# oppo-us-research/PoP-Net

Measured on AMD Instinct MI355X. Metric: depth-frames/sec end-to-end (480x640), higher is better.
Workload: dtype bf16

## Files before the change

popnet_amd/csrc/api.hip:

```cpp
#pragma clang fp contract(off)
#include <cmath>
#include <cstdio>
#include <cstdlib>
#include <cstring>
#include "pn_internal.h"
#include "preproc_pixel.h"

template <typename TIN>
__global__ void preprocess_kernel(const TIN *__restrict__ depth, float *__restrict__ out, int B, int H, int W, int S,
                                  double scale_x, double scale_y, float dmax, float mean, float stdv) {
    const unsigned pix = blockIdx.x * blockDim.x + threadIdx.x;
    if (pix >= (unsigned)(S * S)) return;
    const int b = blockIdx.y;
    const int dy = (int)(pix / (unsigned)S);
    const int dx = (int)(pix - (unsigned)dy * (unsigned)S);
    const size_t gid = (size_t)b * S * S + pix;

    out[gid] = pn_preproc_pixel(depth + (size_t)b * H * W, H, W, dy, dx, scale_x, scale_y, dmax, mean, stdv);
}

PnSwitches pn_read_switches() {
    auto set = [](const char *name) { return getenv(name) != nullptr; };
    auto num = [](const char *name, int unset) { const char *e = getenv(name); return e ? atoi(e) : unset; };
    auto is = [](const char *name, const char *value) { const char *e = getenv(name); return e && !strcmp(e, value); };
    PnSwitches s;
    s.no_conv3 = set("POPNET_NO_CONV3");
    s.conv3_rpg8 = set("POPNET_CONV3_RPG8");
    s.conv3_pt14 = num("POPNET_CONV3_PT14", 0);
    s.conv3_nbuf2 = set("POPNET_CONV3_NBUF2");
    s.generic_c64_off = num("POPNET_GENERIC_C64", 1) == 0;
    if (set("POPNET_CONV4")) s.conv4 = num("POPNET_CONV4", 0) == 0 ? 0 : 1;
    s.no_mix = set("POPNET_NO_MIX");
    s.no_bblock = set("POPNET_NO_BBLOCK");
    s.bblock_x3 = num("POPNET_BBLOCK_X3", 0) != 0;
    s.bb64_static = set("POPNET_BB64_STATIC");
    s.bb64_halves = num("POPNET_BB64_HALVES", 1) == 2 ? 2 : 1;
    s.no_tailfuse = set("POPNET_NO_TAILFUSE");
    s.no_poolfuse = set("POPNET_NO_POOLFUSE");
    s.no_stempool = set("POPNET_NO_STEMPOOL");
    s.no_embed3 = set("POPNET_NO_EMBED3");
    s.train_x3_wide = set("POPNET_TRAIN_X3_WIDE");
    s.train_wgrad_novec = set("POPNET_TRAIN_WGRAD_NOVEC");
    s.trainx_one_stream = num("POPNET_TRAINX_STREAMS", 0) == 1;
    s.trainx_stem_handover = set("POPNET_TRAINX_STEM_HANDOVER");
    s.trainx_stem_gather = is("POPNET_TRAINX_STEM_FWD", "gather");
    s.trainx_stem_bn_separate = is("POPNET_TRAINX_STEM_BN", "separate");
    s.trainx_stem_depth = num("POPNET_TRAINX_STEM_DEPTH", 2);
    s.trainx_pack_gather = is("POPNET_TRAINX_PACK", "gather");
    s.trainx_legacy_wgrad = is("POPNET_TRAINX_WGRAD", "legacy");
    return s;
}

extern "C" {

int pn_abi_version(void) { return PN_ABI_VERSION; }
int pn_build_experiments(void) { return 0; }

pn_ctx *pn_create(int device_id) {
    pn_ctx *ctx = new pn_ctx();
    ctx->device = device_id;
    int ndev = 0;
    hipError_t e = hipGetDeviceCount(&ndev);
    if (e != hipSuccess || device_id < 0 || device_id >= ndev) {
        char buf[256];
        snprintf(buf, sizeof buf, "pn_create: device %d not available (%d devices, %s)", device_id, ndev,
                 hipGetErrorString(e));
        ctx->err = buf;
        ctx->device = -1;
        return ctx;
    }
    hipDeviceProp_t prop;
    if (hipGetDeviceProperties(&prop, device_id) == hipSuccess) ctx->num_cus = prop.multiProcessorCount;
    return ctx;
}

void pn_destroy(pn_ctx *ctx) {
    if (!ctx) return;
    if (ctx->parse_ws) (void)hipFree(ctx->parse_ws);
    pn_parse_big_free(ctx);
    if (ctx->train_ws) (void)hipFree(ctx->train_ws);
    for (void *p : ctx->train_ws_retired) (void)hipFree(p);
    for (auto &e : ctx->train_packs) (void)hipFree(e.buf);
    if (ctx->train_pack_table) (void)hipFree(ctx->train_pack_table);
    delete ctx;
}

int pn_last_error(pn_ctx *ctx, char *buf, size_t buf_len) {
    if (!ctx) return 0;
    if (buf && buf_len) {
        size_t n = ctx->err.size() < buf_len - 1 ? ctx->err.size() : buf_len - 1;
        memcpy(buf, ctx->err.data(), n);
        buf[n] = 0;
    }
    return (int)ctx->err.size();
}

int pn_preprocess(pn_ctx *ctx, const void *depth_dev, int depth_dtype, int B, int H, int W, float *out_dev, int S,
                  float depth_max, float depth_mean, float depth_std, void *hip_stream) {
    if (!ctx) return PN_ERR_INVALID;
    if (ctx->device < 0) return pn_set_error(ctx, PN_ERR_STATE, "context has no device");
    if (!depth_dev || !out_dev || B < 1 || H < 2 || W < 2 || S < 1)
        return pn_set_error(ctx, PN_ERR_INVALID, "pn_preprocess: bad arguments");
    if (W == 2 * S && H == 2 * S)
        return pn_set_error(ctx, PN_ERR_UNSUPPORTED, "pn_preprocess: %dx%d -> %d is an exact 2x decimation, where cv2.resize(INTER_LINEAR) runs INTER_AREA instead: not built", W, H, S);
    const double inv_x = (double)S / (double)W, inv_y = (double)S / (double)H;
    const double scale_x = 1.0 / inv_x, scale_y = 1.0 / inv_y;
    if (B > 65535 || (size_t)S * S > 0x7fffffffu) return pn_set_error(ctx, PN_ERR_INVALID, "pn_preprocess: batch or output size out of range");
    dim3 grid((unsigned)(((size_t)S * S + 255) / 256), (unsigned)B), block(256);
    hipStream_t s = (hipStream_t)hip_stream;
// ... 31 lines not shown
```

popnet_amd/csrc/conv_mfma.hip:

```cpp
#include "pn_internal.h"

int pn_cfg_couts(int cfg) {
    switch (cfg) {
        case PN_CFG_C128: return 128;
        case PN_CFG_C64: return 64;
        case PN_CFG_C64W: return 64;
        case PN_CFG_C32: return 32;
        default: return 16;
    }
}


int pn_cfg_pixels(int cfg) { return cfg == PN_CFG_C128 ? 112 : (cfg == PN_CFG_C64W ? 224 : 128); }

size_t pn_conv_lds_bytes(int prec, int ks, int stride, int pitch, int R) {
    size_t pixb = prec == PN_PREC_BF16 ? 128 : 256;
    size_t rows = (size_t)(R - 1) * stride + ks;
    return rows * pitch * pixb;
}

int pn_launch_conv_part0(pn_ctx *ctx, const ConvLaunch &L, hipStream_t stream);
int pn_launch_conv_part1(pn_ctx *ctx, const ConvLaunch &L, hipStream_t stream);
int pn_launch_conv_part2(pn_ctx *ctx, const ConvLaunch &L, hipStream_t stream);
int pn_launch_conv_part3(pn_ctx *ctx, const ConvLaunch &L, hipStream_t stream);

int pn_launch_conv(pn_ctx *ctx, const ConvLaunch &L, hipStream_t stream) {
    int rc;
    if (L.kern == 4) return pn_launch_conv4(ctx, L, stream);
    if (L.kern == 3) return pn_launch_conv3(ctx, L, stream);
    if ((rc = pn_launch_conv_part0(ctx, L, stream)) != 1) return rc;
    if ((rc = pn_launch_conv_part1(ctx, L, stream)) != 1) return rc;
    if ((rc = pn_launch_conv_part2(ctx, L, stream)) != 1) return rc;
    if ((rc = pn_launch_conv_part3(ctx, L, stream)) != 1) return rc;
    return pn_set_error(ctx, PN_ERR_UNSUPPORTED, "no conv kernel for prec=%d ks=%d stride=%d pitch=%d cfg=%d", L.prec, L.ks,
                        L.stride, L.pitch, L.cfg);
}

int pn_conv_stage_maxpx(int prec, int ks, int stride, int pitch, int cfg) {
    if (cfg == PN_CFG_C64W) return 0;
    const int maxpx = stride != 1 ? 0 : (ks == 1 ? 128 : (pitch <= 32 ? 192 : (pitch <= 64 ? 288 : 360)));
    const int nch = prec == PN_PREC_BF16 ? 8 : 16;
    const int raw = (maxpx * nch + 255) / 256;
    return raw <= 12 ? maxpx : 0;
}
```

popnet_amd/csrc/conv_plan.h:

```cpp
#pragma once
#include <algorithm>
#include "pn_internal.h"

struct ConvGeom {
    int kern = 0, cfg = 0, pitch = 0, R = 0, Wt = 0;
    int wc = 0, wp = 0, nbuf = 0, pt = 7, rpg = 4;
};

inline int pn_pick_pitch(int cols) {
    const int classes[4] = {16, 32, 64, 120};
    for (int c : classes)
        if (cols <= c) return c;
    return -1;
}

inline int pn_pick_cfg(int cout) {
    if (cout % 128 == 0) return PN_CFG_C128;
    if (cout >= 64) return PN_CFG_C64;
    if (cout <= 16) return PN_CFG_C16;
    return PN_CFG_C32;
}

inline void pn_plan_conv_kernel(int prec, int max_batch, int num_cus, int H, int W, int cout, int ks, int stride, int cin_chunks, int wc_min, int nbuf_min,
                                int k4_level, const PnSwitches &sw, ConvGeom &g) {
    g.cfg = pn_pick_cfg(cout);
    {
        int segs = 0, wt = 0, rows = 0, rpg = 4;
        double best = 0;
        for (int sg = (W + 29) / 30; sg <= (W + 15) / 16; ++sg) {
            const int w = (W + sg - 1) / sg;
            for (int gg : {4, 8}) {
                if (gg == 8 && !(w <= 14 && ks == 3 && cout > 64 && sw.conv3_rpg8)) continue;
                const int r = std::min(std::min(H, gg), 112 / w);
                const double util = r * ((double)W / sg) / 112.0;
                if (util > best + 1e-9) { best = util; segs = sg; wt = w; rows = r; rpg = gg; }
            }
        }
        if (prec == PN_PREC_BF16 && stride == 1 && (ks == 3 || ks == 1) && best >= 0.75 && cout > 32 && !sw.no_conv3) {
            g.kern = 3;
            g.wc = std::max(cout > 64 ? 4 : (cout > 32 ? 2 : 1), wc_min);
            const long tiles112 = (long)max_batch * ((H + rows - 1) / rows) * segs;
            g.wp = (g.wc == 2 && rows == 4 && rpg == 4 && tiles112 * ((cout + 63) / 64) >= 1536) ? 2 : 1;
            g.rpg = rpg;
            if (g.wp == 2 && ks == 3 && cin_chunks == 1 && sw.conv3_pt14 == 1) { g.wp = 1; g.pt = 14; g.rpg = 8; }
            if (sw.conv3_pt14 == 2 && ks == 3 && g.wc == 4 && g.wp == 1 && rpg == 4 && rows == 4 && H >= 8) { g.pt = 14; g.rpg = 8; }
            const int hr = rpg * g.wp + ks - 1, ngw = (8 * (hr / 2) + g.wc * g.wp - 1) / (g.wc * g.wp);
            g.nbuf = ((cin_chunks > 1 || nbuf_min == 2) && ks == 3 && ngw <= 18 && sw.conv3_nbuf2) ? 2 : 1;
            g.Wt = wt;
            g.R = std::min(H, rows * g.wp * (g.pt / 7));
            if (ks == 3 && g.wp == 1 && g.pt == 7 && g.rpg == 4 && cout >= 64 && k4_level)
                g.kern = 4;
        }
    }
    if (g.kern == 0 && prec == PN_PREC_BF16 && g.cfg == PN_CFG_C128 && stride == 1) {
        const long blocks128 = (long)max_batch * ((H * W + 111) / 112) * (cout / 128);
        if (blocks128 < num_cus && !sw.generic_c64_off) g.cfg = PN_CFG_C64;
    }
}

inline int pn_plan_conv_tiles(int prec, int H, int W, int ks, int stride, ConvGeom &g, const char **why) {
    const int Ho = (H + 2 * (ks / 2) - ks) / stride + 1, Wo = (W + 2 * (ks / 2) - ks) / stride + 1;
    if (g.kern == 3 || g.kern == 4) { g.pitch = 32; return PN_OK; }
    if (g.cfg == PN_CFG_C64 && ks == 3 && stride == 1 && Wo >= 48 && (long)Ho * Wo >= 2048) g.cfg = PN_CFG_C64W;
    const int BP = pn_cfg_pixels(g.cfg);
    const int wt_cap = std::min(BP, (120 - ks) / stride + 1);
    const int segs = (Wo + wt_cap - 1) / wt_cap;
    g.Wt = (Wo + segs - 1) / segs;
    g.R = std::max(1, std::min(Ho, BP / g.Wt));
    {
        const int maxpx = pn_conv_stage_maxpx(prec, ks, stride, pn_pick_pitch((g.Wt - 1) * stride + ks), g.cfg);
        while (maxpx > 0 && g.R > 1 && ((g.R - 1) * stride + ks) * ((g.Wt - 1) * stride + ks) > maxpx) --g.R;
        if (maxpx > 0 && ((g.R - 1) * stride + ks) * ((g.Wt - 1) * stride + ks) > maxpx) { *why = "halo tile exceeds the staging capacity"; return PN_ERR_UNSUPPORTED; }
    }
    g.pitch = pn_pick_pitch((g.Wt - 1) * stride + ks);
    if (g.pitch < 0) { *why = "halo width has no pitch class"; return PN_ERR_UNSUPPORTED; }
    return PN_OK;
}
```

popnet_amd/csrc/net.hip:

```cpp
#include <cmath>
#include <cstdarg>
#include <cstdio>
#include <algorithm>
#include <cstdlib>
#include <cstring>
#include <map>
#include <memory>
#include <vector>
#include "pn_internal.h"
#include "conv_plan.h"
#include "preproc_pixel.h"

namespace {

struct HostTensor {
    std::vector<int64_t> shape;
    std::vector<float> data;
    size_t numel() const { return data.size(); }
};

struct Buf {
    void *p = nullptr;
    int H = 0, W = 0, C = 0;
    int plane = 0;
// ... 109 lines not shown
int dev_alloc(pn_net *n, void **p, size_t bytes, bool zero) {
    PN_HIP_CHECK(n->ctx, hipMalloc(p, bytes));
    n->dev_allocs.push_back(*p);
    if (zero) PN_HIP_CHECK(n->ctx, hipMemset(*p, 0, bytes));
    return PN_OK;
}

int new_buf(pn_net *n, int H, int W, int C) {
    Buf b;
    b.H = H; b.W = W; b.plane = C; b.C = n->x3 ? 2 * C : C;
    n->bufs.push_back(b);
    return (int)n->bufs.size() - 1;
}

int prepare_conv(pn_net *n, ConvSpec &cs) {
    pn_ctx *ctx = n->ctx;
    const HostTensor *w = find_t(n, cs.w + ".weight");
    if (!w || w->shape.size() != 4)
        return pn_set_error(ctx, PN_ERR_INVALID, "missing conv weight %s.weight", cs.w.c_str());
    const int cout = (int)w->shape[0], cin_ref = (int)w->shape[1], wks = (int)w->shape[2];
    const int ks = cs.embed3 ? 3 : wks;
    if ((cs.embed3 ? wks != 1 : wks != cs.ks) || (int)w->shape[3] != wks || ks != cs.ks)
        return pn_set_error(ctx, PN_ERR_INVALID, "%s.weight: kernel %dx%d, expected %d", cs.w.c_str(), wks, (int)w->shape[3], cs.embed3 ? 1 : cs.ks);
    cs.cout = cout;
    std::vector<int> map = cs.cin_map;
    if (map.empty()) {
        map.resize(cin_ref);
        for (int i = 0; i < cin_ref; ++i) map[i] = i;
    }
    for (int m : map)
        if (m >= cin_ref)
            return pn_set_error(ctx, PN_ERR_INVALID, "%s: input-channel map exceeds Cin=%d", cs.w.c_str(), cin_ref);
    std::vector<int> wsel;
    if (n->x3) {
        const int pc = n->bufs[cs.in_buf].plane;
        if (cs.in_coff != 0 || (int)map.size() > pc)
            return pn_set_error(ctx, PN_ERR_UNSUPPORTED, "%s: bf16x3 convolutions read whole buffers", cs.w.c_str());
        map.resize(pc, -1);
        std::vector<int> m3;
        for (int pl = 0; pl < 3; ++pl)
            for (int i = 0; i < pc; ++i) { m3.push_back(map[i]); wsel.push_back(pl == 2 ? 1 : 0); }
        map.swap(m3);
    }
    const int cin_pad = ((int)map.size() + 63) / 64 * 64;
    map.resize(cin_pad, -1);
    wsel.resize(cin_pad, 0);
    cs.cin_chunks = cin_pad / 64;
    cs.cin = cin_ref;

    std::vector<double> scale(cout, 1.0), shift(cout, 0.0);
    const HostTensor *bias = find_t(n, cs.w + ".bias");
    if (bias && (int)bias->numel() != cout) return pn_set_error(ctx, PN_ERR_INVALID, "%s.bias: bad size", cs.w.c_str());
    for (int o = 0; o < cout; ++o) shift[o] = bias ? bias->data[o] : 0.0;
    if (!cs.bn.empty()) {
        const HostTensor *g = find_t(n, cs.bn + ".weight"), *be = find_t(n, cs.bn + ".bias");
        const HostTensor *mu = find_t(n, cs.bn + ".running_mean"), *var = find_t(n, cs.bn + ".running_var");
        if (!g || !be || !mu || !var || (int)g->numel() != cout || (int)be->numel() != cout ||
            (int)mu->numel() != cout || (int)var->numel() != cout)
            return pn_set_error(ctx, PN_ERR_INVALID, "missing/ill-shaped BatchNorm tensors %s.*", cs.bn.c_str());
        for (int o = 0; o < cout; ++o) {
            double s = (double)g->data[o] / std::sqrt((double)var->data[o] + 1e-5);
            scale[o] = s;
            shift[o] = (shift[o] - (double)mu->data[o]) * s + (double)be->data[o];
        }
    }

    auto wval = [&](int co, int idx, int tap) -> float {
        const int ci = map[idx];
        if (co >= cout || ci < 0) return 0.f;
        if (cs.embed3 && tap != 4) return 0.f;
        const float v = (float)((double)w->data[cs.embed3 ? (size_t)co * cin_ref + ci : ((size_t)co * cin_ref + ci) * (ks * ks) + tap] * scale[co]);
        if (!n->x3) return v;
        uint32_t hb = (uint32_t)f32_to_bf16(v) << 16;
        float hi;
        memcpy(&hi, &hb, 4);
        return wsel[idx] ? v - hi : hi;
    };

    ConvGeom geo;
    geo.pt = cs.pt; geo.rpg = cs.rpg;
    {
        const Buf &ib0 = n->bufs[cs.in_buf];
        pn_plan_conv_kernel(n->prec, n->max_batch, n->ctx->num_cus, ib0.H, ib0.W, cout, ks, cs.stride, cs.cin_chunks, cs.wc_min, cs.nbuf_min, cs.k4_level, n->sw, geo);
    }
    cs.cfg = geo.cfg; cs.kern = geo.kern; cs.wc = geo.wc; cs.wp = geo.wp; cs.nbuf = geo.nbuf; cs.pt = geo.pt; cs.rpg = geo.rpg; cs.Wt = geo.Wt; cs.R = geo.R;
    const int BC = cs.kern == 4 ? 128 : (cs.kern == 3 ? cs.wc * 32 : pn_cfg_couts(cs.cfg));
    const int cout_pad = (cout + BC - 1) / BC * BC;
    const int ctiles = cout_pad / 16;
    const int KK = ks * ks;
    const int ksteps = cs.cin_chunks * KK * 2;
    const size_t fragb = n->prec == PN_PREC_BF16 ? 1024 : 2048;
    const size_t bytes = cs.kern == 4 ? (size_t)(cout_pad / 128) * (ksteps + 3) * 8192
                                      : (size_t)ctiles * ksteps * fragb + 5 * fragb;
    std::vector<unsigned char> host(bytes, 0);
    uint16_t *h16 = reinterpret_cast<uint16_t *>(host.data());
    float *h32 = reinterpret_cast<float *>(host.data());
    if (cs.kern == 4) {
        for (int cbk = 0; cbk < cout_pad / 128; ++cbk)
            for (int hh = 0; hh < cs.cin_chunks * 2; ++hh)
                for (int tap = 0; tap < KK; ++tap)
                    for (int t = 0; t < 8; ++t)
                        for (int lane = 0; lane < 64; ++lane) {
                            const int co = cbk * 128 + pn_conv_row_channel(t, lane & 15, 4), q = lane >> 4;
                            const size_t base = ((((size_t)cbk * (ksteps + 3) + (size_t)hh * KK + tap) * 8 + t) * 64 + lane) * 8;
                            for (int j = 0; j < 8; ++j) h16[base + j] = f32_to_bf16(wval(co, hh * 32 + 8 * q + j, tap));
                        }
    } else
    for (int ct = 0; ct < ctiles; ++ct)
        for (int chunk = 0; chunk < cs.cin_chunks; ++chunk)
            for (int sub = 0; sub < 2; ++sub)
                for (int tap = 0; tap < KK; ++tap) {
                    const size_t kstep = (size_t)(chunk * 2 + sub) * KK + tap;
                    const size_t frag = (size_t)ct * ksteps + kstep;
                    for (int lane = 0; lane < 64; ++lane) {
                        const int co = pn_conv_row_channel(ct, lane & 15, cs.kern == 3 ? 2 : pn_cfg_ct(cs.cfg)), q = lane >> 4;
                        for (int j = 0; j < 8; ++j) {
                            const float v = wval(co, chunk * 64 + sub * 32 + 8 * q + j, tap);
                            if (n->prec == PN_PREC_BF16) h16[(frag * 64 + lane) * 8 + j] = f32_to_bf16(v);
                            else h32[frag * 512 + (size_t)(j >> 2) * 256 + lane * 4 + (j & 3)] = v;
                        }
                    }
                }
    if (int rc = dev_alloc(n, &cs.wpack, bytes, false)) return rc;
    PN_HIP_CHECK(ctx, hipMemcpy(cs.wpack, host.data(), bytes, hipMemcpyHostToDevice));
    std::vector<float> hb(cout_pad, 0.f);
    for (int o = 0; o < cout; ++o) hb[o] = (float)shift[o];
    if (int rc = dev_alloc(n, (void **)&cs.bias, hb.size() * 4, false)) return rc;
    PN_HIP_CHECK(ctx, hipMemcpy(cs.bias, hb.data(), hb.size() * 4, hipMemcpyHostToDevice));

    const Buf &ib = n->bufs[cs.in_buf];
    const int Ho = (ib.H + 2 * (ks / 2) - ks) / cs.stride + 1, Wo = (ib.W + 2 * (ks / 2) - ks) / cs.stride + 1;
    {
        const char *why = "";
        if (int rc = pn_plan_conv_tiles(n->prec, ib.H, ib.W, ks, cs.stride, geo, &why)) return pn_set_error(ctx, rc, "%s: %s", cs.w.c_str(), why);
        cs.cfg = geo.cfg; cs.pitch = geo.pitch; cs.Wt = geo.Wt; cs.R = geo.R;
    }
    cs.flops = 2.0 * Ho * Wo * (double)cout * cin_ref * (cs.embed3 ? 1 : KK);
    if (cs.out_buf >= 0) {
        const Buf &ob = n->bufs[cs.out_buf];
        if (ob.H != Ho || ob.W != Wo) return pn_set_error(ctx, PN_ERR_INVALID, "%s: output buffer is %dx%d, conv gives %dx%d", cs.w.c_str(), ob.H, ob.W, Ho, Wo);
    }
    return PN_OK;
}

int add_conv(pn_net *n, const std::string &w, const std::string &bn, int ks, int stride, int in_buf, int in_coff,
             int out_buf, int out_coff, int act, int res_buf = -1, int nchw_slot = -1,
             std::vector<int> cin_map = std::vector<int>()) {
    ConvSpec cs;
    cs.w = w; cs.bn = bn; cs.ks = ks; cs.stride = stride;
    cs.in_buf = in_buf; cs.in_coff = in_coff;
    cs.out_buf = out_buf; cs.out_coff = out_coff;
    cs.res_buf = res_buf; cs.act = act; cs.nchw_slot = nchw_slot;
    cs.cin_map = std::move(cin_map);
    n->convs.push_back(cs);
    return (int)n->convs.size() - 1;
}

void harmonize_level(pn_net *n, const std::vector<int> &ids) {
    {
        bool k4 = false;
        for (int id : ids) {
            const ConvSpec &c = n->convs[id];
            const HostTensor *w = find_t(n, c.w + ".weight");
            if (w && w->shape.size() == 4 && c.ks == 3 && c.stride == 1 && w->shape[0] >= 64 && (n->x3 || std::max<int64_t>(w->shape[1], (int64_t)c.cin_map.size()) > 64)) k4 = true;
        }
        long blocks = 0;
// ... 475 lines not shown
    for (auto &st : n->steps) {
        if (st.type != Step::CONV) continue;
        const ConvSpec &c0 = n->convs[st.conv_ids[0]];
        const int BC = c0.kern == 4 ? 128 : (c0.kern == 3 ? c0.wc * 32 : pn_cfg_couts(c0.cfg));
        st.host_probs.clear();
        int max_blocks = 0;
        bool two_bufs = false, has_tail = false, pool_tail = false;
        for (int id : st.conv_ids) {
            const ConvSpec &cs = n->convs[id];
            const Buf &ib = n->bufs[cs.in_buf];
            ConvProblem P;
            memset(&P, 0, sizeof P);
            const size_t es = n->esize();
            (void)es;
            P.in = ib.p;
            P.wpack = cs.wpack;
            P.bias = cs.bias;
            P.B = B; P.H = ib.H; P.W = ib.W;
            P.Ho = (ib.H + 2 * (cs.ks / 2) - cs.ks) / cs.stride + 1;
            P.Wo = (ib.W + 2 * (cs.ks / 2) - cs.ks) / cs.stride + 1;
            P.cin_chunks = cs.cin_chunks;
            P.in_cs = ib.C; P.in_coff = cs.in_coff;
            if (n->x3 && ib.plane % 64)
                return pn_set_error(n->ctx, PN_ERR_UNSUPPORTED, "bf16x3: input plane of %d channels is not a multiple of 64 (the K loop wraps to the hi plane per 64-channel chunk)", ib.plane);
            P.in_wrap = n->x3 ? 2 * (ib.plane / 64) : (1 << 20);
            P.cout = cs.cout;
            if (cs.out_buf >= 0) { P.out = n->bufs[cs.out_buf].p; P.out_cs = n->bufs[cs.out_buf].C; P.out_coff = cs.out_coff; P.split = n->x3 ? n->bufs[cs.out_buf].plane : 0; }
            if (cs.res_buf >= 0) { P.res = n->bufs[cs.res_buf].p; P.res_cs = n->bufs[cs.res_buf].C; P.res_coff = cs.res_coff; P.res_split = n->x3 ? n->bufs[cs.res_buf].plane : 0; }
            if (cs.nchw_slot >= 0) P.out_nchw = n->nchw_ptr[cs.nchw_slot];
            P.act = cs.act;
            P.yolo_naf = 5 + 3 * n->num_parts;
            P.R = cs.R;
            P.Wt = cs.Wt;
            P.tiles_x = (P.Wo + cs.Wt - 1) / cs.Wt;
            P.tiles_per_img = ((P.Ho + cs.R - 1) / cs.R) * P.tiles_x;
            P.cout_blocks = (cs.cout + BC - 1) / BC;
            P.nblocks = B * P.tiles_per_img * P.cout_blocks;
            if (cs.kern == 4) P.nblocks = ((B * P.tiles_per_img + 1) / 2) * P.cout_blocks;
            P.ksteps = cs.cin_chunks * cs.ks * cs.ks * 2;
            P.ks = cs.ks;
            P.lds_buf_bytes = (int)pn_conv_lds_bytes(n->prec, cs.ks, cs.stride, cs.pitch, cs.R);
            P.lds_two = (cs.cin_chunks > 1 && 2 * (size_t)P.lds_buf_bytes <= 160 * 1024) ? 1 : 0;
            P.in_zero_off = (unsigned)((size_t)n->max_batch * ib.H * ib.W * ib.C * es);
            if (cs.pool_tail) {
                const Buf &pb = n->bufs[cs.pool_out_buf];
                P.tiles_x = (pb.W + 6) / 7;
                P.tiles_per_img = ((pb.H + 2) / 3) * P.tiles_x;
                P.nblocks = B * P.tiles_per_img * P.cout_blocks;
                P.tail_out = pb.p; P.tail_out_cs = pb.C; P.tail_out_coff = cs.pool_out_coff;
                P.tail_split = n->x3 ? pb.plane : 0;
                P.out = nullptr;
                pool_tail = true;
            }
            if (cs.tail_conv >= 0) {
                const ConvSpec &tb = n->convs[cs.tail_conv];
                P.tail_w = cs.tail_wpack; P.tail_bias = cs.tail_bias; P.tail_cout = tb.cout; P.tail_act = tb.act;
                if (tb.out_buf >= 0) { P.tail_out = n->bufs[tb.out_buf].p; P.tail_out_cs = n->bufs[tb.out_buf].C; P.tail_out_coff = tb.out_coff; }
                if (tb.nchw_slot >= 0) P.tail_nchw = n->nchw_ptr[tb.nchw_slot];
                P.out = nullptr;
                has_tail = true;
            }
            if (P.lds_two) two_bufs = true;
            max_blocks = std::max(max_blocks, P.nblocks);
            st.host_probs.push_back(P);
        }
        st.launch.prec = n->prec;
        st.launch.ks = c0.ks; st.launch.stride = c0.stride; st.launch.pitch = c0.pitch; st.launch.cfg = c0.cfg;
        st.launch.nprob = (int)st.host_probs.size();
        st.launch.max_blocks = max_blocks;
        st.launch.lds_bytes = pn_conv_lds_bytes(n->prec, c0.ks, c0.stride, c0.pitch, c0.R) * (two_bufs ? 2 : 1);
        st.launch.kern = c0.kern; st.launch.wc = c0.wc; st.launch.wp = c0.wp; st.launch.nbuf = c0.nbuf; st.launch.pt = c0.pt; st.launch.rpg = c0.rpg;
        if (c0.kern == 3) st.launch.lds_bytes = pn_conv3_lds_bytes(c0.ks, c0.wp, c0.nbuf, c0.rpg);
        st.launch.tail = (c0.kern == 3 && has_tail) ? 1 : (c0.kern == 3 && pool_tail) ? 2 : 0;
        st.launch.mix = 0;
        if (c0.kern == 3) {
            for (int id : st.conv_ids) {
                const ConvSpec &cs = n->convs[id];
                if (cs.ks != c0.ks || (cs.tail_conv >= 0) != (c0.tail_conv >= 0)) st.launch.mix = 1;
                st.launch.lds_bytes = std::max(st.launch.lds_bytes, pn_conv3_lds_bytes(cs.ks, cs.wp, cs.nbuf, cs.rpg));
            }
            if (st.launch.tail == 1) st.launch.lds_bytes = std::max<size_t>(st.launch.lds_bytes, 4 * 7 * 1024 + 1024);
            if (st.launch.tail == 2 && n->x3) st.launch.lds_bytes = std::max<size_t>(st.launch.lds_bytes, 2 * 4 * 7 * 1024);
        }
        if (c0.kern == 4) st.launch.lds_bytes = 0;
        st.launch.probs_dev = st.dev_probs;
        PN_HIP_CHECK(n->ctx, hipMemcpyAsync(st.dev_probs, st.host_probs.data(), st.host_probs.size() * sizeof(ConvProblem),
                                            hipMemcpyHostToDevice, stream));
    }
    n->last_B = B;
    for (int i = 0; i < 4; ++i) n->last_nchw[i] = n->nchw_ptr[i];
    return PN_OK;
}

std::string step_label(const pn_net *n, const Step &st) {
    if (st.type == Step::STEM) {
        if (st.stem_pool_buf >= 0) return "stem7x7_pool_kernel";
        if (st.stem_cin > 1) return "conv2d_forward+nchw_relu_to_nhwc_kernel";
        if (n->prec == PN_PREC_F32) return "stem7x7_kernel";
        return n->x3 ? "stem7x7_mfma_kernel<x3>" : "stem7x7_mfma_kernel";
    }
    if (st.type == Step::POOL) return pn_pool_kernel_label(st.mode, n->x3);
    if (st.type == Step::BBLOCK) return n->x3 ? "bb64x3_kernel" : "bb64_kernel";
    const ConvSpec &c0 = n->convs[st.conv_ids[0]];
    bool mix = false;
    for (int id : st.conv_ids) {
        const ConvSpec &cs = n->convs[id];
        if (cs.ks != c0.ks || (cs.tail_conv >= 0) != (c0.tail_conv >= 0)) mix = true;
    }
    return pn_conv_kernel_label(n->prec, c0.kern, mix, c0.ks, c0.stride, c0.pitch, c0.cfg, c0.wc, c0.wp, c0.nbuf, c0.pt, c0.rpg);
}

int run_forward(pn_net *n, const float *x, int B, hipStream_t stream, int nsteps = -1) {
    pn_ctx *ctx = n->ctx;
    if (!n->finalized) return pn_set_error(ctx, PN_ERR_STATE, "pn_net_finalize has not been called");
    if (B < 1 || B > n->max_batch) return pn_set_error(ctx, PN_ERR_INVALID, "batch %d outside [1, %d]", B, n->max_batch);
    bool dirty = B != n->last_B;
    for (int i = 0; i < 4; ++i) dirty |= n->nchw_ptr[i] != n->last_nchw[i];
    if (dirty) {
        if (n->locked)
            return pn_set_error(ctx, PN_ERR_STATE, "net is locked at batch %d (pn_net_lock): a forward with another batch size or other output buffers would rewrite descriptors a captured graph still reads", n->last_B);
        if (int rc = refresh_problems(n, B, stream)) return rc;
    }
    if (n->tickets_suspect) {
        for (auto &st : n->steps)
            if (st.type == Step::BBLOCK && st.bb_tickets) PN_HIP_CHECK(ctx, hipMemsetAsync(st.bb_tickets, 0, 256, stream));
        n->tickets_suspect = false;
    }
    for (size_t si = 0; si < n->steps.size(); ++si) {
        if ((int)si == nsteps) break;
        Step &st = n->steps[si];
        int rc = PN_OK;
        pn_net::ProfRec *pr = nullptr;
        if (n->profiling) {
            if (n->prof_used == n->prof.size()) {
                pn_net::ProfRec r;
                PN_HIP_CHECK(ctx, hipEventCreate(&r.a));
                PN_HIP_CHECK(ctx, hipEventCreate(&r.b));
                n->prof.push_back(r);
            }
            pr = &n->prof[n->prof_used++];
            pr->kind = (int)st.type;
            pr->flops = 0;
            pr->label.clear();
            if (st.type == Step::CONV) {
                for (int id : st.conv_ids) pr->flops += n->convs[id].flops * B;
                pr->label = step_label(n, st);
            }
            if (st.type == Step::BBLOCK) {
                pr->kind = (int)Step::CONV;
                pr->flops = (n->convs[st.bb_a].flops + n->convs[st.bb_b].flops) * B;
                pr->label = step_label(n, st);
            }
            PN_HIP_CHECK(ctx, hipEventRecord(pr->a, stream));
        }
        if (st.type == Step::STEM && st.stem_pool_buf >= 0) {
            const Buf &ob = n->bufs[st.out_buf], &pb = n->bufs[st.stem_pool_buf];
            rc = pn_launch_stem_pool(ctx, x, st.stem_wfrag, st.stem_b, pb.p, B, n->in_h, n->in_w, ob.H, ob.W, pb.C, stream, n->frame_src.frames ? &n->frame_src : nullptr);
        } else if (st.type == Step::STEM && st.stem_cin > 1) {
            const Buf &ob = n->bufs[st.out_buf];
            if (n->frame_src.frames) return pn_set_error(ctx, PN_ERR_UNSUPPORTED, "the frames-in forward takes single-channel depth frames (input_dim = 1)");
            rc = pn_conv2d_forward(ctx, x, st.stem_w, st.stem_b, st.stem_scratch, B, st.stem_cin, n->in_h, n->in_w, 64, 7, 2, 3, 0, (void *)stream);
            if (!rc) rc = pn_launch_nchw_relu_to_nhwc(ctx, n->prec, st.stem_scratch, ob.p, B, ob.H, ob.W, 64, ob.C, n->x3 ? ob.plane : 0, stream);
        } else if (st.type == Step::STEM) {
            const Buf &ob = n->bufs[st.out_buf];
            rc = pn_launch_stem(ctx, n->x3 ? PN_PREC_BF16X3 : n->prec, x, st.stem_w, st.stem_wfrag, st.stem_b, ob.p, B, n->in_h, n->in_w, ob.H, ob.W, ob.C, n->x3 ? ob.plane : 0, stream,
                                n->frame_src.frames ? &n->frame_src : nullptr);
        } else if (st.type == Step::POOL) {
// ... 325 lines not shown
```

popnet_amd/csrc/pn_internal.h:

```cpp
#pragma once
#include <hip/hip_runtime.h>
#include <stdint.h>
#include <string>
#include <vector>
#include "../../include/popnet_hip.h"

struct pn_ctx {
    int device = 0;
    std::string err;
    int num_cus = 256;
    void *parse_ws = nullptr;
    size_t parse_ws_bytes = 0;
    bool parse_ws_fixed = false;
    int parse_last_b = 0;
    void *parse_big = nullptr;
    void *train_ws = nullptr;
    size_t train_ws_bytes = 0;
    bool train_ws_keep = false;
    std::vector<void *> train_ws_retired;
    bool train_lds_attr = false;
    bool train_x3 = false;
    struct PackEntry { const float *w; int Cout, Cin, flip, x3; void *buf; size_t bytes; bool fresh; };
    bool train_pack_cache = false;
    std::vector<PackEntry> train_packs;
    void *train_pack_table = nullptr;
    size_t train_pack_table_entries = 0;
    size_t train_pack_table_cap = 0;
    unsigned train_pack_blocks = 0;
};

struct PnSwitches {
    bool no_conv3 = false;
    bool conv3_rpg8 = false;
    int conv3_pt14 = 0;
    bool conv3_nbuf2 = false;
    bool generic_c64_off = false;
    int conv4 = -1;
    bool no_mix = false;
    bool no_bblock = false;
    bool bblock_x3 = false;
    bool bb64_static = false;
    int bb64_halves = 1;
    bool no_tailfuse = false;
    bool no_poolfuse = false;
    bool no_stempool = false;
    bool no_embed3 = false;
    bool train_x3_wide = false;
    bool train_wgrad_novec = false;
    bool trainx_one_stream = false;
    bool trainx_stem_handover = false;
    bool trainx_stem_gather = false;
    bool trainx_stem_bn_separate = false;
    int trainx_stem_depth = 2;
    bool trainx_pack_gather = false;
    bool trainx_legacy_wgrad = false;
};
PnSwitches pn_read_switches();

int pn_set_error(pn_ctx *ctx, int code, const char *fmt, ...);
void pn_parse_big_free(pn_ctx *ctx);
int pn_train_ws(pn_ctx *ctx, size_t bytes, void **out);
const char *pn_dgrad_strided_plan(int N, int Cin, int H, int W, int ks, unsigned *grid_x, unsigned *grid_y);

#define PN_HIP_CHECK(ctx, expr)                                                              \
    do {                                                                                     \
        hipError_t _e = (expr);                                                              \
        if (_e != hipSuccess)                                                                \
            return pn_set_error((ctx), PN_ERR_HIP, "%s failed: %s (%s:%d)", #expr,           \
                                hipGetErrorString(_e), __FILE__, __LINE__);                  \
    } while (0)

struct PnLdsAttr { size_t bytes[64] = {}; };
inline int pn_lds_attr(pn_ctx *ctx, PnLdsAttr &st, const void *kern, size_t bytes) {
    const int d = ctx->device >= 0 && ctx->device < 64 ? ctx->device : 0;
    if (st.bytes[d] >= bytes) return PN_OK;
    PN_HIP_CHECK(ctx, hipFuncSetAttribute(kern, hipFuncAttributeMaxDynamicSharedMemorySize, (int)bytes));
    st.bytes[d] = bytes;
    return PN_OK;
}

enum pn_act {
    PN_ACT_NONE = 0,
    PN_ACT_RELU = 1,
    PN_ACT_LEAKY = 2,
    PN_ACT_SIG_PM2 = 3,
    PN_ACT_SIG = 4,
    PN_ACT_YOLO = 5
};

struct ConvProblem {
    const void *in;
    const void *wpack;
    const float *bias;
    const void *res;
    void *out;
    float *out_nchw;
    int B, H, W;
    int Ho, Wo;
    int cin_chunks;
    int in_cs, in_coff;
    int cout;
    int out_cs, out_coff;
    int res_cs, res_coff;
    int act;
    int yolo_naf;
    int R;
    int Wt, tiles_x;
    int tiles_per_img;
    int cout_blocks;
    int nblocks;
    int ksteps;
    int ks;
    int lds_buf_bytes;
    int lds_two;
    unsigned in_zero_off;
    int split;
    int res_split;
    int in_wrap;
    const void *tail_w;
    const float *tail_bias;
    void *tail_out;
    float *tail_nchw;
    int tail_cout, tail_act, tail_out_cs, tail_out_coff;
    int tail_split;
};

enum pn_conv_cfg {
    PN_CFG_C128 = 0,
    PN_CFG_C64 = 1,
    PN_CFG_C32 = 2,
    PN_CFG_C16 = 3,
    PN_CFG_C64W = 4
};
int pn_cfg_couts(int cfg);
inline int pn_cfg_ct(int cfg) { return cfg == PN_CFG_C16 ? 1 : 2; }
inline int pn_conv_row_channel(int tile, int row, int CT) {
    return (tile / CT) * CT * 16 + 4 * CT * (row >> 2) + 4 * (tile % CT) + (row & 3);
}
int pn_cfg_pixels(int cfg);

struct ConvLaunch {
    int prec;
    int ks;
    int stride;
    int pitch;
    int cfg;
    int kern = 0, wc = 0, wp = 0, nbuf = 0, pt = 7, rpg = 4;
    int tail = 0;
    int mix = 0;
    int nprob;
    int max_blocks;
    size_t lds_bytes;
    const ConvProblem *probs_dev;
};
int pn_launch_conv(pn_ctx *ctx, const ConvLaunch &L, hipStream_t stream);
inline std::string pn_conv_kernel_label(int prec, int kern, bool mix, int ks, int stride, int pitch, int cfg, int wc, int wp, int nbuf, int pt, int rpg) {
    char lb[96];
    if (kern == 4) snprintf(lb, sizeof lb, "conv4_kernel");
    else if (kern == 3 && mix) snprintf(lb, sizeof lb, "conv3_mix_kernel");
    else if (kern == 3) snprintf(lb, sizeof lb, "conv3_kernel<%d, %d, %d, %d, %d, %d>", ks, wc, wp, nbuf, pt, rpg);
    else snprintf(lb, sizeof lb, "conv_mfma_kernel<%d, %d, %d, %d, %d>", prec, ks, stride, pitch, cfg);
    return lb;
}
inline std::string pn_pool_kernel_label(int mode, bool split) {
    char lb[48];
    snprintf(lb, sizeof lb, "pool_kernel<%d%s>", mode, split ? ", split" : "");
    return lb;
}
int pn_launch_conv3(pn_ctx *ctx, const ConvLaunch &L, hipStream_t stream);
int pn_launch_conv4(pn_ctx *ctx, const ConvLaunch &L, hipStream_t stream);

struct BBProblem {
    const void *in;
    void *out;
    const void *wpack;
    const float *bias1, *bias2;
    int B, H, W;
    int in_cs, in_coff, out_cs, out_coff;
    int Wt, tiles_x, tiles_per_img, ntiles;
    unsigned in_zero_off;
    int in_split, out_split;
    int *tickets;
    int halves;
};
int pn_launch_bb64(pn_ctx *ctx, const BBProblem &P, hipStream_t stream);
int pn_launch_bb64x3(pn_ctx *ctx, const BBProblem &P, hipStream_t stream);
size_t pn_conv3_lds_bytes(int ks, int WP, int nbuf, int rpg = 4);
size_t pn_conv_lds_bytes(int prec, int ks, int stride, int pitch, int R);
int pn_conv_stage_maxpx(int prec, int ks, int stride, int pitch, int cfg);

struct PnFrameSrc;
int pn_launch_stem_pool(pn_ctx *ctx, const float *x, const void *wfrag, const float *bias, void *out, int B, int H, int W, int Ho, int Wo,
                        int out_cs, hipStream_t stream, const PnFrameSrc *src);
struct PnFrameSrc;
int pn_launch_stem(pn_ctx *ctx, int prec, const float *x, const float *w, const void *wfrag, const float *bias,
                   void *out, int B, int H, int W, int Ho, int Wo, int out_cs, int split, hipStream_t stream, const PnFrameSrc *src = nullptr);

int pn_launch_pool(pn_ctx *ctx, int prec, int mode, const void *in, void *out, int B, int H, int W,
                   int C, int in_cs, int out_cs, int out_coff, int in_split, int out_split, hipStream_t stream);

int pn_stem_forward_planes(pn_ctx *ctx, const float *x_dev, const float *w_dev, void *y_planes, int cs, int split, int f32, int N, int Cin, int H, int W, int Cout,
                           int ks, int stride, int pad, int gather, hipStream_t s);
struct PnStemBn {
    const void *x; int x_cs, x_split;
    const float *mean, *invstd, *k1, *k2, *k3, *scale, *shift;
    int act;
};
int pn_stem_wgrad_planes(pn_ctx *ctx, const float *x_dev, const void *dy_planes, int cs, int split, int f32, const PnStemBn *bn, float *dw_dev, int N, int Cin, int H,
                         int W, int Cout, int ks, int stride, int pad, int depth, hipStream_t s);
int pn_launch_nchw_relu_to_nhwc(pn_ctx *ctx, int prec, const float *in, void *out, int B, int H, int W, int C, int out_cs, int split, hipStream_t stream);
int pn_launch_nhwc_to_nchw(pn_ctx *ctx, int prec, const void *in, float *out, int B, int H, int W,
                           int C, int in_cs, int in_coff, int split, hipStream_t stream);
```

Before: 68480.

## Add opt-in specialized MFMA kernel for narrow 3x3 head convolutions

Adds a dedicated bf16 3x3 stride-1 kernel (headk) for layers with at most 16 output channels and narrow width. It stages the whole halo tile and all weight steps into LDS per input-channel chunk, then runs a software-pipelined MFMA loop with explicit scheduling barriers, and writes NHWC and/or NCHW output with a fused activation. The aim is to avoid the generic kernel's overhead on small head layers. It is only selected when POPNET_HEADK is set. A separate unconditional tweak bumps the LDS pitch from 16 to 32 for 1x1 stride-1 convolutions, which changes the layout of those layers.

```diff
diff --git a/popnet_amd/csrc/api.hip b/popnet_amd/csrc/api.hip
--- a/popnet_amd/csrc/api.hip
+++ b/popnet_amd/csrc/api.hip
@@ -25,6 +25,7 @@
     auto is = [](const char *name, const char *value) { const char *e = getenv(name); return e && !strcmp(e, value); };
     PnSwitches s;
     s.no_conv3 = set("POPNET_NO_CONV3");
+    s.headk = num("POPNET_HEADK", 0) != 0;
     s.conv3_rpg8 = set("POPNET_CONV3_RPG8");
     s.conv3_pt14 = num("POPNET_CONV3_PT14", 0);
     s.conv3_nbuf2 = set("POPNET_CONV3_NBUF2");
diff --git a/popnet_amd/csrc/conv_mfma.hip b/popnet_amd/csrc/conv_mfma.hip
--- a/popnet_amd/csrc/conv_mfma.hip
+++ b/popnet_amd/csrc/conv_mfma.hip
@@ -26,6 +26,7 @@
 
 int pn_launch_conv(pn_ctx *ctx, const ConvLaunch &L, hipStream_t stream) {
     int rc;
+    if (L.kern == 5) return pn_launch_headk(ctx, L, stream);
     if (L.kern == 4) return pn_launch_conv4(ctx, L, stream);
     if (L.kern == 3) return pn_launch_conv3(ctx, L, stream);
     if ((rc = pn_launch_conv_part0(ctx, L, stream)) != 1) return rc;
diff --git a/popnet_amd/csrc/conv_plan.h b/popnet_amd/csrc/conv_plan.h
--- a/popnet_amd/csrc/conv_plan.h
+++ b/popnet_amd/csrc/conv_plan.h
@@ -58,9 +58,18 @@
     }
 }
 
+inline bool pn_plan_headk(int prec, int H, int W, int cout, int ks, int stride, const PnSwitches &sw, ConvGeom &g) {
+    if (prec != PN_PREC_BF16 || ks != 3 || stride != 1 || cout > 16 || W > 30 || g.kern != 0 || sw.no_conv3 || !sw.headk) return false;
+    g.kern = 5;
+    g.cfg = PN_CFG_C16;
+    g.Wt = W;
+    g.R = std::min(H, 4);
+    return true;
+}
+
 inline int pn_plan_conv_tiles(int prec, int H, int W, int ks, int stride, ConvGeom &g, const char **why) {
     const int Ho = (H + 2 * (ks / 2) - ks) / stride + 1, Wo = (W + 2 * (ks / 2) - ks) / stride + 1;
-    if (g.kern == 3 || g.kern == 4) { g.pitch = 32; return PN_OK; }
+    if (g.kern == 3 || g.kern == 4 || g.kern == 5) { g.pitch = 32; return PN_OK; }
     if (g.cfg == PN_CFG_C64 && ks == 3 && stride == 1 && Wo >= 48 && (long)Ho * Wo >= 2048) g.cfg = PN_CFG_C64W;
     const int BP = pn_cfg_pixels(g.cfg);
     const int wt_cap = std::min(BP, (120 - ks) / stride + 1);
@@ -74,5 +83,6 @@
     }
     g.pitch = pn_pick_pitch((g.Wt - 1) * stride + ks);
     if (g.pitch < 0) { *why = "halo width has no pitch class"; return PN_ERR_UNSUPPORTED; }
+    if (ks == 1 && stride == 1 && g.pitch == 16) g.pitch = 32;
     return PN_OK;
 }
diff --git a/popnet_amd/csrc/headk_inst.hip b/popnet_amd/csrc/headk_inst.hip
--- /dev/null
+++ b/popnet_amd/csrc/headk_inst.hip
@@ -0,0 +1,3 @@
+#include "headk_kernel.h"
+
+int pn_launch_headk(pn_ctx *ctx, const ConvLaunch &L, hipStream_t stream) { return headk_launch(ctx, L, stream); }
diff --git a/popnet_amd/csrc/headk_kernel.h b/popnet_amd/csrc/headk_kernel.h
--- /dev/null
+++ b/popnet_amd/csrc/headk_kernel.h
@@ -0,0 +1,161 @@
+#pragma once
+#include "conv3_kernel.h"
+
+constexpr int PNH_PT = 2;
+constexpr int PNH_HR = 6;
+constexpr int PNH_IMG = 2 * PNH_HR * 32 * 64;
+constexpr int PNH_WSTEPS = 18;
+constexpr int PNH_LDS = PNH_IMG + PNH_WSTEPS * 1024;
+
+__global__ __launch_bounds__(256, 3) void headk_kernel(const ConvProblem *__restrict__ probs) {
+    typedef __bf16 T;
+    typedef Elem<PN_PREC_BF16>::Frag Frag;
+    constexpr int PT = PNH_PT, HR = PNH_HR, IMG = PNH_IMG, PITCH = 32;
+    constexpr int NG = 8 * (HR / 2);
+    constexpr int NDMA = NG + PNH_WSTEPS;
+    constexpr int NGW = (NDMA + 3) / 4;
+    extern __shared__ __attribute__((aligned(16))) char smem[];
+
+    const ConvProblem &P = probs[blockIdx.y];
+    if ((int)blockIdx.x >= P.nblocks) return;
+    int bx;
+    {
+        const int nb = P.nblocks, xcd = blockIdx.x & 7, idx = blockIdx.x >> 3;
+        const int qq = nb >> 3, rr = nb & 7;
+        bx = (xcd < rr ? xcd * (qq + 1) : rr * (qq + 1) + (xcd - rr) * qq) + idx;
+    }
+    const int tid = threadIdx.x;
+    const int lane = tid & 63;
+    const int wave = __builtin_amdgcn_readfirstlane(tid >> 6);
+    const int c = lane & 15, q = lane >> 4;
+
+    const int tile = bx % P.tiles_per_img;
+    const int b = bx / P.tiles_per_img;
+    const int ty = tile / P.tiles_x, tx = tile - ty * P.tiles_x;
+    const int oy0 = ty * P.R, ox0 = tx * P.Wt;
+    const int R = min(P.R, P.Ho - oy0);
+    const int Wo = P.Wo;
+    const int Wc = min(P.Wt, Wo - ox0);
+    const int npix = R * Wc;
+    const int HC = Wc + 2;
+    const int iy0 = oy0 - 1, ix0 = ox0 - 1;
+    const float inv_wc = 1.0f / (float)Wc;
+    const int nchunks = P.cin_chunks;
+
+    gcptr img = (gcptr)P.in + ((size_t)b * P.H * P.W * P.in_cs + P.in_coff) * 2;
+    const unsigned zero_rel = P.in_zero_off - (unsigned)(((size_t)b * P.H * P.W * P.in_cs + P.in_coff) * 2);
+    const int row_b = P.W * P.in_cs * 2, col_b = P.in_cs * 2;
+    gcptr wsrc = (gcptr)P.wpack + lane * 16;
+    auto stage = [&](int chunk) {
+#pragma unroll
+        for (int j = 0; j < NGW; ++j) {
+            const int n = wave * NGW + j;
+            if (n < NG) {
+                const int hh = n / (2 * HR), rr = (n - hh * 2 * HR) >> 1, gg = n & 1;
+                const int px = gg * 16 + (lane >> 2);
+                const int iy = iy0 + rr;
+                const bool inb = px < HC && (unsigned)(ix0 + px) < (unsigned)P.W && (unsigned)iy < (unsigned)P.H;
+                const unsigned off = (unsigned)(iy * row_b + (ix0 + px) * col_b + hh * 64 + (lane & 3) * 16);
+                const unsigned zrel = zero_rel - (unsigned)(chunk * 128);
+                pn_glds16(img + chunk * 128 + (inb ? off : zrel),
+                          (unsigned)__builtin_amdgcn_readfirstlane(hh * (IMG / 2) + (rr * PITCH + gg * 16) * 64));
+            } else if (n < NDMA) {
+                const int s = n - NG;
+                pn_glds16(wsrc + (size_t)(chunk * PNH_WSTEPS + s) * 1024, (unsigned)__builtin_amdgcn_readfirstlane(IMG + s * 1024));
+            }
+        }
+    };
+    stage(0);
+
+    int baddr[PT];
+#pragma unroll
+    for (int pt = 0; pt < PT; ++pt) {
+        const int slot = (wave * PT + pt) * 16 + c;
+        const int s = slot < npix ? slot : 0;
+        const int ry = (int)(((float)s + 0.5f) * inv_wc);
+        const int rx = s - ry * Wc;
+        baddr[pt] = q * 16 + (ry * PITCH + rx) * 64;
+    }
+    f32x4 acc[PT];
+#pragma unroll
+    for (int pt = 0; pt < PT; ++pt) acc[pt] = f32x4{0.f, 0.f, 0.f, 0.f};
+    const int cw = 4 * q;
+    const f32x4 b4 = *reinterpret_cast<const PN_GLOBAL f32x4 *>((const PN_GLOBAL float *)P.bias + cw);
+
+    asm volatile("s_waitcnt vmcnt(0)" ::: "memory");
+    __syncthreads();
+
+    constexpr int NITEM = PNH_WSTEPS * PT, DB = 6;
+    for (int chunk = 0; chunk < nchunks; ++chunk) {
+#define PNH_OFF(j) ((((j) / PT) / 9) * (IMG / 2) + (((((j) / PT) % 9) / 3) * PITCH + (((j) / PT) % 3)) * 64)
+        Frag aw[PNH_WSTEPS], bq[DB];
+#pragma unroll
+        for (int s = 0; s < PNH_WSTEPS; ++s) aw[s] = read_b_frag<PN_PREC_BF16>(smem + IMG + s * 1024, lane * 16);
+#pragma unroll
+        for (int j = 0; j < DB - 1; ++j) bq[j] = read_b_frag<PN_PREC_BF16>(smem + PNH_OFF(j), baddr[j % PT]);
+        __builtin_amdgcn_sched_barrier(0);
+#pragma unroll
+        for (int j = 0; j < NITEM; ++j) {
+            const int jr = j + DB - 1;
+            if (jr < NITEM) bq[jr % DB] = read_b_frag<PN_PREC_BF16>(smem + PNH_OFF(jr), baddr[jr % PT]);
+            acc[j % PT] = mma(aw[j / PT], bq[j % DB], acc[j % PT]);
+            if (jr < NITEM) __builtin_amdgcn_sched_group_barrier(0x100, 1, 0);
+            __builtin_amdgcn_sched_group_barrier(0x008, 1, 0);
+        }
+#undef PNH_OFF
+        if (chunk + 1 < nchunks) {
+            __syncthreads();
+            stage(chunk + 1);
+            asm volatile("s_waitcnt vmcnt(0)" ::: "memory");
+            __syncthreads();
+        }
+    }
+
+    const int cout = P.cout, act = P.act, naf = P.yolo_naf;
+    if (cw >= cout) return;
+    const bool full = cw + 4 <= cout;
+    PN_GLOBAL T *out_base = P.out ? (PN_GLOBAL T *)P.out + P.out_coff + cw : nullptr;
+    PN_GLOBAL float *nchw = (PN_GLOBAL float *)P.out_nchw;
+    const int out_cs = P.out_cs, Ho = P.Ho;
+    const int pix0 = (b * Ho + oy0) * Wo + ox0;
+#pragma unroll
+    for (int pt = 0; pt < PT; ++pt) {
+        const int slot = (wave * PT + pt) * 16 + c;
+        if (slot >= npix) continue;
+        const int ry = (int)(((float)slot + 0.5f) * inv_wc);
+        const int rx = slot - ry * Wc;
+        const int opix = pix0 + ry * Wo + rx;
+        float v[4];
+#pragma unroll
+        for (int k = 0; k < 4; ++k) {
+            v[k] = acc[pt][k] + b4[k];
+            if (cw + k < cout) v[k] = pn_activate(v[k], act, cw + k, naf);
+        }
+        if (out_base) {
+            PN_GLOBAL T *op = out_base + (unsigned)(opix * out_cs);
+            T ov[4];
+#pragma unroll
+            for (int k = 0; k < 4; ++k) ov[k] = (T)v[k];
+            if (full) {
+                *reinterpret_cast<PN_GLOBAL u32x2 *>(op) = *reinterpret_cast<u32x2 *>(ov);
+            } else {
+#pragma unroll
+                for (int k = 0; k < 4; ++k)
+                    if (cw + k < cout) op[k] = ov[k];
+            }
+        }
+        if (nchw) {
+            const size_t hw = (size_t)Ho * Wo;
+            PN_GLOBAL float *np = nchw + ((size_t)b * cout + cw) * hw + (size_t)(oy0 + ry) * Wo + (ox0 + rx);
+#pragma unroll
+            for (int k = 0; k < 4; ++k)
+                if (cw + k < cout) np[(size_t)k * hw] = v[k];
+        }
+    }
+}
+
+static int headk_launch(pn_ctx *ctx, const ConvLaunch &L, hipStream_t stream) {
+    hipLaunchKernelGGL(headk_kernel, dim3(L.max_blocks, L.nprob), dim3(256), PNH_LDS, stream, L.probs_dev);
+    PN_HIP_CHECK(ctx, hipGetLastError());
+    return PN_OK;
+}
diff --git a/popnet_amd/csrc/net.hip b/popnet_amd/csrc/net.hip
--- a/popnet_amd/csrc/net.hip
+++ b/popnet_amd/csrc/net.hip
@@ -215,6 +215,7 @@
     {
         const Buf &ib0 = n->bufs[cs.in_buf];
         pn_plan_conv_kernel(n->prec, n->max_batch, n->ctx->num_cus, ib0.H, ib0.W, cout, ks, cs.stride, cs.cin_chunks, cs.wc_min, cs.nbuf_min, cs.k4_level, n->sw, geo);
+        if (!n->x3) pn_plan_headk(n->prec, ib0.H, ib0.W, cout, ks, cs.stride, n->sw, geo);
     }
     cs.cfg = geo.cfg; cs.kern = geo.kern; cs.wc = geo.wc; cs.wp = geo.wp; cs.nbuf = geo.nbuf; cs.pt = geo.pt; cs.rpg = geo.rpg; cs.Wt = geo.Wt; cs.R = geo.R;
     const int BC = cs.kern == 4 ? 128 : (cs.kern == 3 ? cs.wc * 32 : pn_cfg_couts(cs.cfg));
@@ -856,7 +857,7 @@
             if (st.launch.tail == 1) st.launch.lds_bytes = std::max<size_t>(st.launch.lds_bytes, 4 * 7 * 1024 + 1024);
             if (st.launch.tail == 2 && n->x3) st.launch.lds_bytes = std::max<size_t>(st.launch.lds_bytes, 2 * 4 * 7 * 1024);
         }
-        if (c0.kern == 4) st.launch.lds_bytes = 0;
+        if (c0.kern == 4 || c0.kern == 5) st.launch.lds_bytes = 0;
         st.launch.probs_dev = st.dev_probs;
         PN_HIP_CHECK(n->ctx, hipMemcpyAsync(st.dev_probs, st.host_probs.data(), st.host_probs.size() * sizeof(ConvProblem),
                                             hipMemcpyHostToDevice, stream));
diff --git a/popnet_amd/csrc/pn_internal.h b/popnet_amd/csrc/pn_internal.h
--- a/popnet_amd/csrc/pn_internal.h
+++ b/popnet_amd/csrc/pn_internal.h
@@ -31,6 +31,7 @@
 
 struct PnSwitches {
     bool no_conv3 = false;
+    bool headk = false;
     bool conv3_rpg8 = false;
     int conv3_pt14 = 0;
     bool conv3_nbuf2 = false;
@@ -157,6 +158,7 @@
 inline std::string pn_conv_kernel_label(int prec, int kern, bool mix, int ks, int stride, int pitch, int cfg, int wc, int wp, int nbuf, int pt, int rpg) {
     char lb[96];
     if (kern == 4) snprintf(lb, sizeof lb, "conv4_kernel");
+    else if (kern == 5) snprintf(lb, sizeof lb, "headk_kernel");
     else if (kern == 3 && mix) snprintf(lb, sizeof lb, "conv3_mix_kernel");
     else if (kern == 3) snprintf(lb, sizeof lb, "conv3_kernel<%d, %d, %d, %d, %d, %d>", ks, wc, wp, nbuf, pt, rpg);
     else snprintf(lb, sizeof lb, "conv_mfma_kernel<%d, %d, %d, %d, %d>", prec, ks, stride, pitch, cfg);
@@ -169,6 +171,7 @@
 }
 int pn_launch_conv3(pn_ctx *ctx, const ConvLaunch &L, hipStream_t stream);
 int pn_launch_conv4(pn_ctx *ctx, const ConvLaunch &L, hipStream_t stream);
+int pn_launch_headk(pn_ctx *ctx, const ConvLaunch &L, hipStream_t stream);
 
 struct BBProblem {
     const void *in;
```

Result: no change. 68340 (-0.2%).
